# jopohl/urh

Hardware: NVIDIA H100
Metric: MSamples/s IQ demod+digitize (complex64) (higher is better)
Workload: dtype f32

## Files before the change

urh_b200/csrc/dense_f32.cuh:

```cuda
#pragma once
#include "dense.cuh"

struct SrcQad {
    static constexpr bool BINARY = false;
    template <typename T> __device__ __forceinline__ static int cls(T s, const UrhClassify& C, float) { return urh_classify((float)s, C); }
    template <typename T> __device__ __forceinline__ static void bits(T, const UrhClassify&, float, bool& nz, bool& ab) { nz = false; ab = false; }
    template <typename T> __device__ __forceinline__ static bool above(T, float) { return false; }
};
struct SrcQad2 {
    static constexpr bool BINARY = true;
    template <typename T> __device__ __forceinline__ static int cls(T s, const UrhClassify& C, float thr0) {
        const int c = ((float)s <= thr0) ? 0 : 1;
        return ((float)s == C.noise_value) ? -1 : c;
    }
    template <typename T> __device__ __forceinline__ static void bits(T s, const UrhClassify& C, float thr0, bool& nz, bool& ab) {
        nz = (float)s == C.noise_value;
        ab = !((float)s <= thr0) && !nz;
    }
    template <typename T> __device__ __forceinline__ static bool above(T s, float thr0) { return !((float)s <= thr0); }
};
struct SrcAbove {
    static constexpr bool BINARY = true;
    template <typename T> __device__ __forceinline__ static int cls(T s, const UrhClassify&, float thr0) { return (s > (T)thr0) ? 1 : 0; }
    template <typename T> __device__ __forceinline__ static void bits(T s, const UrhClassify&, float thr0, bool& nz, bool& ab) { nz = false; ab = s > (T)thr0; }
    template <typename T> __device__ __forceinline__ static bool above(T s, float thr0) { return s > (T)thr0; }
};
struct SrcCenter {
    static constexpr bool BINARY = true;
    template <typename T> __device__ __forceinline__ static int cls(T s, const UrhClassify&, float thr0) { return (s <= (T)thr0) ? 0 : 1; }
    template <typename T> __device__ __forceinline__ static void bits(T s, const UrhClassify&, float thr0, bool& nz, bool& ab) { nz = false; ab = !(s <= (T)thr0); }
    template <typename T> __device__ __forceinline__ static bool above(T s, float thr0) { return !(s <= (T)thr0); }
};

struct UrhSpec {
    const float* tg;
    float* margin;
    int64_t lo, hi;
    unsigned int* redone;
};

template <typename T> struct UrhVec2;
template <> struct UrhVec2<float> { typedef float2 type; };
template <> struct UrhVec2<double> { typedef double2 type; };

template <typename SRC, typename T>
__global__ void __launch_bounds__(URH_WARPS_PER_BLOCK * 32)
k_dense_f32(const T* __restrict__ x, int64_t n, int vec_in, const __grid_constant__ UrhClassify cls, int tol,
            UrhTileSummary* __restrict__ tiles, uint32_t* __restrict__ staging, int stage_cap,
            int16_t* __restrict__ init_cls, int cls_of_zero, const float* __restrict__ d_thr0 = nullptr,
            const UrhTileStats* __restrict__ tile_stats = nullptr, const UrhSpec spec = UrhSpec{}) {
    const float thr0 = d_thr0 ? *d_thr0 : cls.thr[0];
    if (d_thr0) cls_of_zero = (0.0f <= thr0) ? 0 : 1;
    const int lane = threadIdx.x & 31;
    const int64_t tile = (int64_t)blockIdx.x * URH_WARPS_PER_BLOCK + (threadIdx.x >> 5);
    const int64_t tile_start = tile * URH_TILE;
    if (tile_start >= n) return;
    const int tile_len = (int)((n - tile_start) < URH_TILE ? (n - tile_start) : URH_TILE);
    const int iters = (tile_len + 63) >> 6;
    if (tile_stats && tile_stats[tile].all_noise) {
        if (lane == 0) {
            UrhTileSummary s;
            s.first_cls = -1; s.last_cls = -1; s.head_len = tile_len; s.tail_len = tile_len; s.ncand = 0;
            tiles[tile] = s;
            if (tile_start == 0 && init_cls) *init_cls = (int16_t)-1;
        }
        return;
    }
    if (tile >= spec.lo && tile < spec.hi) {
        if (spec.margin[tile] > fabsf(__fsub_rn(thr0, *spec.tg))) return;
        if (lane == 0) atomicAdd(spec.redone, 1u);
    }
    UrhRunTracker rt;
    rt.init(tol, staging + tile * (int64_t)stage_cap);
    if (vec_in && tile_len == URH_TILE) {
        typedef typename UrhVec2<T>::type V;
        const V* p = (const V*)(x + tile_start) + lane;
        constexpr int ITERS = URH_TILE / 64;
        const bool no_noise = SRC::BINARY && tile_stats && cls.noise_value <= -4.0f && tile_stats[tile].cnt == URH_TILE;
        V cur[4], nxt[4];
#pragma unroll
        for (int j = 0; j < 4; j++) cur[j] = __ldg(p + j * 32);
        if (tile_start == 0 && lane == 0 && init_cls) *init_cls = (int16_t)(((float)cur[0].x == cls.noise_value) ? -1 : cls_of_zero);
        if (SRC::BINARY) {
            UrhTileResolve tr;
            tr.init();
#pragma unroll 1
            for (int it = 0; it < ITERS; it += 4) {
                if (it + 4 < ITERS) {
#pragma unroll
                    for (int j = 0; j < 4; j++) nxt[j] = __ldg(p + (it + 4 + j) * 32);
                }
                if (no_noise) {
#pragma unroll
                    for (int j = 0; j < 4; j++)
                        tr.keep(it + j, 0u, __ballot_sync(URH_FULL_MASK, SRC::template above<T>(cur[j].x, thr0)), 0u,
                                __ballot_sync(URH_FULL_MASK, SRC::template above<T>(cur[j].y, thr0)), lane);
                } else {
#pragma unroll
                    for (int j = 0; j < 4; j++) {
                        bool nx, ax, ny, ay;
                        SRC::template bits<T>(cur[j].x, cls, thr0, nx, ax);
                        SRC::template bits<T>(cur[j].y, cls, thr0, ny, ay);
                        tr.keep(it + j, __ballot_sync(URH_FULL_MASK, nx), __ballot_sync(URH_FULL_MASK, ax), __ballot_sync(URH_FULL_MASK, ny),
                                __ballot_sync(URH_FULL_MASK, ay), lane);
                    }
                }
#pragma unroll
                for (int j = 0; j < 4; j++) cur[j] = nxt[j];
            }
            tr.finish(tol, staging + tile * (int64_t)stage_cap, tiles + tile, lane);
            return;
        }
#pragma unroll 1
        for (int it = 0; it < ITERS; it += 4) {
            if (it + 4 < ITERS) {
#pragma unroll
                for (int j = 0; j < 4; j++) nxt[j] = __ldg(p + (it + 4 + j) * 32);
            }
#pragma unroll
            for (int j = 0; j < 4; j++)
                rt.feed(it + j, SRC::template cls<T>(cur[j].x, cls, thr0), SRC::template cls<T>(cur[j].y, cls, thr0), true, true, lane);
#pragma unroll
            for (int j = 0; j < 4; j++) cur[j] = nxt[j];
        }
        rt.finish(tile_len, tiles + tile, lane);
        return;
    }
    for (int it = 0; it < iters; it += 2) {
        T a0 = 0, a1 = 0, b0 = 0, b1 = 0;
        const int64_t pa = tile_start + (int64_t)it * 64 + 2 * lane;
        const int64_t pb = pa + 64;
        if (vec_in && pa + 1 < n) {
            const typename UrhVec2<T>::type v = __ldg((const typename UrhVec2<T>::type*)(x + pa));
            a0 = v.x; a1 = v.y;
        } else {
            if (pa < n) a0 = __ldg(x + pa);
            if (pa + 1 < n) a1 = __ldg(x + pa + 1);
        }
        const bool has_b = it + 1 < iters;
        if (has_b) {
            if (vec_in && pb + 1 < n) {
                const typename UrhVec2<T>::type v = __ldg((const typename UrhVec2<T>::type*)(x + pb));
                b0 = v.x; b1 = v.y;
            } else {
                if (pb < n) b0 = __ldg(x + pb);
                if (pb + 1 < n) b1 = __ldg(x + pb + 1);
            }
        }
        if (pa == 0 && init_cls) *init_cls = (int16_t)(((float)a0 == cls.noise_value) ? -1 : cls_of_zero);
        rt.feed(it, SRC::template cls<T>(a0, cls, thr0), SRC::template cls<T>(a1, cls, thr0), pa < n, pa + 1 < n, lane);
        if (has_b) rt.feed(it + 1, SRC::template cls<T>(b0, cls, thr0), SRC::template cls<T>(b1, cls, thr0), pb < n, pb + 1 < n, lane);
    }
    rt.finish(tile_len, tiles + tile, lane);
}
```

urh_b200/csrc/digitize.cu:

```cuda
#include "dense.cuh"
#include "scan.cuh"
#include "sparse.cuh"
#ifndef URH_FAST_MIN_BLOCKS
#define URH_FAST_MIN_BLOCKS 4
#endif
#include "fsk_fast.cuh"
#include "dense_f32.cuh"
#include "stream_ring.cuh"

#include <math.h>
#include <stdlib.h>


template <int DT, int MOD, bool DIGITIZE>
__device__ __forceinline__ void dense_iq_tile(const void* __restrict__ iq, int64_t n, const UrhDemodParams& dp, float* __restrict__ qad_out,
                                              int vec_in, int vec_out, const UrhClassify& cls, int tol, UrhTileSummary* __restrict__ tiles,
                                              uint32_t* __restrict__ staging, int stage_cap, int16_t* __restrict__ init_cls, int cls_of_zero,
                                              int64_t tile, int has_halo, UrhTileStats* __restrict__ tile_stats, const UrhFine& fine,
                                              unsigned int* s_fine, unsigned int* g_fine) {
    const int lane = threadIdx.x & 31;
    const int64_t tile_start = tile * URH_TILE;
    const int tile_len = (int)((n - tile_start) < URH_TILE ? (n - tile_start) : URH_TILE);
    const int iters = (tile_len + 63) >> 6;

// ... 874 lines not shown
        const StreamSizes z = stream_sizes(n, dtype, tolerance, sc->chunk_samples, sc->ring, URH_STREAM_ENTRY_DEMOD_CENTER_DIGITIZE);
        scs = z.cs;
        URH_CHECK(ring.init(ctx, sc->ring, sc->ring * r256(z.src_slot)));
        const int64_t slot = r256(z.src_slot);
        URH_CHECK(stream_run(ctx, n, scs, ring, (const char*)sc->h_iq, urh_iq_bytes(dtype), true, ring.mem, slot, sc->h_qad, d_qad_out,
                             [&](int64_t, int64_t s0, int64_t s1, int s) {
                                 return stream_dense_iq<false>(ctx, dtype, mod_type, ring.mem, slot, n, dp, d_qad_out, cls, 0, nullptr, s0, s1, s,
                                                               ts, fine);
                             }, true));
    }
    cls.noise_value = urh_noise_value(mod_type);
    cls.order = 2;
    const int tol = tolerance;
    const int cap = stage_cap_for(tol);
    UrhTileSummary* tiles = nullptr;
    uint32_t* staging = nullptr;
    int16_t* d_init = nullptr;
    if (!sc) {
        URH_CHECK(urh_arena(ctx, (size_t)ntiles, &tiles));
        URH_CHECK(urh_arena(ctx, (size_t)ntiles * cap, &staging));
        URH_CHECK(urh_arena(ctx, 8, &d_init));
    }
    const bool speculate = !sharded && !h_iq && !sc && mod_type == URH_MOD_FSK && dtype == URH_DT_F32 &&
                           getenv("URH_B200_NO_SPECULATE") == nullptr;
    UrhSpec spec = {};
    if (speculate) {
        float* tg;
        URH_CHECK(urh_arena(ctx, 1, &tg));
        URH_CHECK(urh_arena(ctx, 1, &spec.redone));
        URH_CHECK(urh_arena(ctx, (size_t)ntiles, &spec.margin));
        spec.tg = tg;
        const char* forced = getenv("URH_B200_SPECULATE_GUESS");
        URH_LAUNCH(ctx, k_speculate_guess, 1, URH_GUESS_THREADS, 0, (const float2*)d_iq, n, dp.noise_sqrd, forced ? 1 : 0,
                   forced ? strtof(forced, nullptr) : 0.0f, tg, spec.redone);
    }
    int chunk_no = 0;
    for (int64_t t0 = 0; t0 < (sc ? 0 : ntiles); t0 += chunk_tiles, chunk_no++) {
        const int64_t t1 = (t0 + chunk_tiles < ntiles) ? t0 + chunk_tiles : ntiles;
        if (h_iq) {
            const int64_t s0 = t0 * URH_TILE, s1 = (t1 * URH_TILE < n) ? t1 * URH_TILE : n;
            cudaEvent_t ev = ctx->ev_copy[chunk_no & 1];
            URH_CUDA(ctx, cudaMemcpyAsync((char*)d_iq + (size_t)s0 * sample_bytes, (const char*)h_iq + (size_t)s0 * sample_bytes,
                                          (size_t)(s1 - s0) * sample_bytes, cudaMemcpyHostToDevice, ctx->copy_stream[0]));
            URH_CUDA(ctx, cudaEventRecord(ev, ctx->copy_stream[0]));
            URH_CUDA(ctx, cudaStreamWaitEvent(ctx->stream, ev, 0));
        }
        if (mod_type == URH_MOD_ASK)
            URH_CHECK((launch_dense_iq_m<URH_MOD_ASK, false>(ctx, dtype, d_iq, n, dp, d_qad_out, cls, 0, nullptr, nullptr, 0, nullptr, 0, has_halo, ts, t0, t1, fine)));
        else
            URH_CHECK((launch_dense_iq_m<URH_MOD_FSK, false>(ctx, dtype, d_iq, n, dp, d_qad_out, cls, tol, tiles, staging, cap, nullptr, 0, has_halo,
                                                             ts, t0, t1, fine, speculate ? &spec : nullptr)));
    }
    CenterPlan* plan = nullptr;
    URH_CHECK(urh_center_chain(ctx, d_qad_out, n, ts, max_size, sharded ? ctx->nccl_rank : 0, sharded ? ctx->nccl_world : 1,
                               fine.gh ? &fine : nullptr, &plan));
    const float* d_centerf;
    const double* d_center;
    const int* d_state;
    urh_center_plan_result(ctx, plan, &d_centerf, &d_center, &d_state);
    int64_t rows = 0;
    if (sc) {
        URH_CUDA(ctx, cudaMemcpyAsync(ctx->h_mail + 40, d_center, sizeof(double), cudaMemcpyDeviceToHost, ctx->stream));
        URH_CUDA(ctx, cudaMemcpyAsync(ctx->h_mail + 41, d_state, sizeof(int), cudaMemcpyDeviceToHost, ctx->stream));
        URH_CHECK(urh_center_plan_certify_stats(ctx, plan, ctx->h_mail + 42));
        URH_CUDA(ctx, cudaMemcpyAsync(ctx->h_mail + 45, (const int64_t*)ctx->center_prefix + ntiles, sizeof(int64_t), cudaMemcpyDeviceToHost,
                                      ctx->stream));
        URH_CUDA(ctx, cudaStreamSynchronize(ctx->stream));
        int st0 = 0;
        memcpy(&st0, ctx->h_mail + 41, sizeof(int));
        if (st0 == 1) {
            StreamDigitizer dz;
            URH_CHECK(dz.init(ctx, n, scs, tol, mod_type == URH_MOD_ASK, samples_per_symbol));
            for (int64_t s0 = 0; s0 < n; s0 += scs) {
                const int64_t s1 = s0 + scs < n ? s0 + scs : n;
                URH_CHECK(stream_dense_qad(ctx, d_qad_out + s0, s0, s1, cls, dz, d_centerf, ts));
                URH_CHECK(dz.finish(ctx, s0, s1));
            }
            rows = dz.rows;
        }
        *sc->kept = ctx->h_mail[45];
    } else {
        URH_CUDA(ctx, cudaMemsetAsync(d_init, 0, 16, ctx->stream));
        const int vec_in = (((uintptr_t)d_qad_out % 8) == 0) ? 1 : 0;
        URH_LAUNCH(ctx, (k_dense_f32<SrcQad2, float>), (unsigned)urh_div_up(ntiles, URH_WARPS_PER_BLOCK), URH_WARPS_PER_BLOCK * 32, 0,
                   (const float*)d_qad_out, n, vec_in, cls, tol, tiles, staging, cap, d_init, 0, d_centerf, (const UrhTileStats*)ts, spec);
        URH_CUDA(ctx, cudaMemcpyAsync(ctx->h_mail + 40, d_center, sizeof(double), cudaMemcpyDeviceToHost, ctx->stream));
        URH_CUDA(ctx, cudaMemcpyAsync(ctx->h_mail + 41, d_state, sizeof(int), cudaMemcpyDeviceToHost, ctx->stream));
        URH_CHECK(urh_center_plan_certify_stats(ctx, plan, ctx->h_mail + 42));
        ctx->h_mail[46] = 0;
        if (speculate) URH_CUDA(ctx, cudaMemcpyAsync(ctx->h_mail + 46, spec.redone, sizeof(unsigned int), cudaMemcpyDeviceToHost, ctx->stream));
        if (sharded)
            URH_CHECK(urh_finish_shard(ctx, n, tol, mod_type == URH_MOD_ASK, samples_per_symbol, tiles, staging, cap, d_init, global_offset, n_total, &rows));
        else
            URH_CHECK(urh_finish_local(ctx, n, tol, mod_type == URH_MOD_ASK, samples_per_symbol, tiles, staging, cap, d_init, &rows));
    }
    memcpy(center, ctx->h_mail + 40, sizeof(double));
    int st = 0;
    memcpy(&st, ctx->h_mail + 41, sizeof(int));
    *center_state = st;
    ctx->center_cert[0] = ctx->h_mail[42];
    ctx->center_cert[1] = fine.gh ? URH_FINE_NB : 0;
    ctx->center_cert[2] = ctx->h_mail[44];
    const int64_t redone = (spec.hi > spec.lo) ? ctx->h_mail[46] : 0;
    ctx->spec_stats[0] = spec.hi - spec.lo;
    ctx->spec_stats[1] = spec.hi - spec.lo - redone;
    ctx->spec_stats[2] = redone;
    if (st != 1) {
        ctx->pulses_k = 0;
        rows = 0;
    }
    *k = rows;
    return URH_OK;
}

extern "C" int urh_speculate_stats(urh_ctx* ctx, int64_t* h_out3) {
    for (int i = 0; i < 3; i++) h_out3[i] = ctx->spec_stats[i];
    return URH_OK;
}

extern "C" int urh_demod_center_digitize(urh_ctx* ctx, const void* d_iq, int dtype, int64_t n, float noise_mag, int mod_type,
                                         uint16_t tolerance, uint32_t samples_per_symbol, int64_t max_size, float* d_qad_out,
                                         double* center, int* center_state, int64_t* k) {
    return demod_center_digitize_impl(ctx, d_iq, dtype, n, 0, noise_mag, mod_type, tolerance, samples_per_symbol, max_size, d_qad_out, false,
                                      0, n, center, center_state, k);
}

extern "C" int urh_demod_center_digitize_host(urh_ctx* ctx, const void* h_iq, int dtype, int64_t n, float noise_mag, int mod_type,
                                              uint16_t tolerance, uint32_t samples_per_symbol, int64_t max_size, int64_t chunk_samples,
                                              void* d_iq_scratch, float* d_qad_out, double* center, int* center_state, int64_t* k) {
    if (!h_iq || !d_iq_scratch) return URH_ERR_INVALID;
    URH_CUDA(ctx, cudaEventRecord(ctx->ev_comp[0], ctx->stream));
    URH_CUDA(ctx, cudaStreamWaitEvent(ctx->copy_stream[0], ctx->ev_comp[0], 0));
    return demod_center_digitize_impl(ctx, d_iq_scratch, dtype, n, 0, noise_mag, mod_type, tolerance, samples_per_symbol, max_size, d_qad_out,
                                      false, 0, n, center, center_state, k, h_iq, chunk_samples > 0 ? chunk_samples : ((int64_t)1 << 24));
}

extern "C" int urh_shard_demod_center_digitize_host(urh_ctx* ctx, const void* h_iq, int dtype, int64_t n, int has_halo, float noise_mag,
                                                    int mod_type, uint16_t tolerance, uint32_t samples_per_symbol, int64_t max_size,
                                                    int64_t chunk_samples, void* d_iq_scratch, float* d_qad_out, int64_t global_offset,
                                                    int64_t n_total, double* center, int* center_state, int64_t* k) {
    if (!h_iq || !d_iq_scratch) return URH_ERR_INVALID;
    URH_CUDA(ctx, cudaEventRecord(ctx->ev_comp[0], ctx->stream));
    URH_CUDA(ctx, cudaStreamWaitEvent(ctx->copy_stream[0], ctx->ev_comp[0], 0));
    return demod_center_digitize_impl(ctx, d_iq_scratch, dtype, n, has_halo, noise_mag, mod_type, tolerance, samples_per_symbol, max_size,
                                      d_qad_out, true, global_offset, n_total, center, center_state, k, h_iq,
                                      chunk_samples > 0 ? chunk_samples : ((int64_t)1 << 24));
}

extern "C" int urh_shard_demod_center_digitize(urh_ctx* ctx, const void* d_iq, int dtype, int64_t n, int has_halo, float noise_mag,
                                               int mod_type, uint16_t tolerance, uint32_t samples_per_symbol, int64_t max_size,
                                               float* d_qad_out, int64_t global_offset, int64_t n_total, double* center,
                                               int* center_state, int64_t* k) {
    return demod_center_digitize_impl(ctx, d_iq, dtype, n, has_halo, noise_mag, mod_type, tolerance, samples_per_symbol, max_size, d_qad_out,
                                      true, global_offset, n_total, center, center_state, k);
}

extern "C" int urh_afp_demod_stream(urh_ctx* ctx, const void* h_iq, int dtype, int64_t n, float noise_mag, int mod_type, int64_t chunk_samples,
                                    int ring, float* h_qad) {
    if (!h_iq || !h_qad) return URH_ERR_INVALID;
    URH_CHECK(stream_check(ctx, n, ring, mod_type, dtype, true));
    urh_arena_reset(ctx);
    const StreamSizes z = stream_sizes(n, dtype, 0, chunk_samples, ring, URH_STREAM_ENTRY_AFP_DEMOD);
    StreamRing R;
    URH_CHECK(R.init(ctx, ring, z.ring_bytes));
    char* d_src = R.mem;
    float* d_qad = (float*)(R.mem + ring * r256(z.src_slot));
    const UrhDemodParams dp = make_demod_params(noise_mag, mod_type, dtype);
// ... 276 lines not shown
```

urh_b200/csrc/finish.cu:

```cuda
#include "sparse.cuh"
#include "tilescan.cuh"

#include <limits.h>

#define CLS_NONE INT_MIN

struct __align__(16) CandAgg {
    int64_t cnt;
    int32_t last_cls;
    int32_t pad;
};
struct CandOp {
    __device__ __forceinline__ CandAgg operator()(const CandAgg& a, const CandAgg& b) const {
        CandAgg r;
        r.cnt = a.cnt + b.cnt;
        r.last_cls = (b.last_cls != CLS_NONE) ? b.last_cls : a.last_cls;
        r.pad = 0;
        return r;
    }
};
struct __align__(16) FireAgg {
    int64_t fired;
    int64_t last_pos;
};
struct FireOp {
    __device__ __forceinline__ FireAgg operator()(const FireAgg& a, const FireAgg& b) const {
        FireAgg r;
        r.fired = a.fired + b.fired;
        r.last_pos = (b.last_pos >= 0) ? b.last_pos : a.last_pos;
        return r;
    }
};

struct ScanRunCarry {
    const UrhTileSummary* tiles;
    int64_t n;
    RunCarry* carry;
    __device__ __forceinline__ RunCarry load(int64_t t) const {
        const int64_t rem = n - t * URH_TILE;
        const int tile_len = rem < URH_TILE ? (int)rem : URH_TILE;
        const UrhTileSummary s = tiles[t];
        RunCarry r;
        r.len = s.tail_len;
        r.cls = s.last_cls;
        r.flags = (s.head_len == tile_len) ? 1 : 0;
        return r;
    }
    __device__ __forceinline__ void post(int64_t t, const RunCarry& excl, const RunCarry&) const { carry[t] = excl; }
};

struct ScanCandidates {
    const UrhTileSummary* tiles;
    const uint32_t* staging;
    int stage_cap;
    const RunCarry* carry;
    const RunCarry* xcarry;
    int tol;
    int32_t* head_rel;
    int32_t* prev_cls;
    __device__ __forceinline__ CandAgg load(int64_t t) const {
        const UrhTileSummary s = tiles[t];
        RunCarry c = carry[t];
        if (xcarry) c = RunCarryOp()(*xcarry, c);
        int64_t start_len = 0;
        if (!(c.flags & 2) && c.cls == s.first_cls) start_len = c.len;
        int32_t rel = -1;
        if (start_len <= tol && (int64_t)tol < start_len + s.head_len) rel = (int32_t)(tol - start_len);
        head_rel[t] = rel;
        CandAgg r;
        r.cnt = (int64_t)s.ncand + (rel >= 0 ? 1 : 0);
        r.last_cls = CLS_NONE;
        if (s.ncand > 0) r.last_cls = (int32_t)(staging[t * (int64_t)stage_cap + s.ncand - 1] & 0xffffu) - 1;
        else if (rel >= 0) r.last_cls = s.first_cls;
        r.pad = 0;
        return r;
    }
    __device__ __forceinline__ void post(int64_t t, const CandAgg& excl, const CandAgg&) const { prev_cls[t] = excl.last_cls; }
};

struct ScanFirings {
    const UrhTileSummary* tiles;
    const uint32_t* staging;
    int stage_cap;
    const int32_t* head_rel;
    const int32_t* prev_cls;
    const int16_t* d_prev0;
    int64_t global_offset;
    int64_t* row_off;
    int64_t* prev_fired;
    __device__ __forceinline__ FireAgg load(int64_t t) const {
        const UrhTileSummary s = tiles[t];
        int prev = prev_cls[t];
        if (prev == CLS_NONE) prev = *d_prev0;
        const int64_t base = t * URH_TILE + global_offset;
        FireAgg r;
        r.fired = 0;
        r.last_pos = -1;
        const int32_t rel = head_rel[t];
        if (rel >= 0) {
            const int c = s.first_cls;
            if (c != prev) { r.fired++; r.last_pos = base + rel; }
            prev = c;
        }
        const uint32_t* st = staging + t * (int64_t)stage_cap;
        for (int j = 0; j < s.ncand; j++) {
            const uint32_t v = st[j];
            const int c = (int)(v & 0xffffu) - 1;
            if (c != prev) { r.fired++; r.last_pos = base + (v >> 16); }
            prev = c;
        }
        return r;
    }
    __device__ __forceinline__ void post(int64_t t, const FireAgg& excl, const FireAgg&) const {
        row_off[t] = excl.fired;
        prev_fired[t] = excl.last_pos;
    }
};

__global__ void __launch_bounds__(256) k_finish_rows(const UrhTileSummary* __restrict__ tiles, const uint32_t* __restrict__ staging,
                                                    int stage_cap, const int32_t* __restrict__ head_rel, const int32_t* __restrict__ prev_cls,
                                                    const int16_t* __restrict__ d_prev0, const int64_t* __restrict__ row_off,
                                                    const int64_t* __restrict__ prev_fired, const int64_t* __restrict__ d_xprev_fired,
                                                    int64_t ntiles, int64_t global_offset, int64_t n_total, int tol, int is_ask, int64_t sps,
                                                    int emit_tail, int64_t row_base, int64_t* __restrict__ out, int64_t cap_rows,
                                                    int64_t* __restrict__ d_out) {
    const int64_t t = (int64_t)blockIdx.x * blockDim.x + threadIdx.x;
    if (t >= ntiles) return;
    const UrhTileSummary s = tiles[t];
    int prev = prev_cls[t];
    if (prev == CLS_NONE) prev = *d_prev0;
    int64_t pp = prev_fired[t];
    if (pp < 0) pp = *d_xprev_fired;
    int64_t idx = row_off[t];
    const int64_t base = t * URH_TILE + global_offset;
    auto fire = [&](int64_t p, int c) {
        if (c != prev) {
            const int64_t rec = (pp >= 0) ? (p - pp) : (p + 1 - tol);
            int64_t st = prev;
            if (is_ask && st == -1 && rec < sps) st = 0;
            if (idx < cap_rows) *((longlong2*)out + idx) = make_longlong2(st, rec);
            idx++;
            pp = p;
        }
        prev = c;
    };
    const int32_t rel = head_rel[t];
    if (rel >= 0) fire(base + rel, s.first_cls);
    const uint32_t* st = staging + t * (int64_t)stage_cap;
    for (int j = 0; j < s.ncand; j++) {
        const uint32_t v = st[j];
        fire(base + (v >> 16), (int)(v & 0xffffu) - 1);
    }
    if (t == ntiles - 1) {
        const int64_t fired = idx;
        if (emit_tail && (is_ask || row_base + fired < n_total)) {
            if (idx < cap_rows) *((longlong2*)out + idx) = make_longlong2(prev, (pp >= 0) ? (n_total - 1 - pp) : (n_total - tol));
            idx++;
        }
        d_out[0] = idx;
        d_out[1] = fired;
    }
}

struct ScanMergeRows {
    const int64_t* raw;
    int64_t rows;
    int64_t n_total;
    int has_tail;
    int64_t* out;
    int64_t* d_k;
    const int64_t* prev_last;
    int64_t row_base;
    __device__ __forceinline__ int64_t load(int64_t r) const {
        if (r == 0) return (prev_last && raw[0] == *prev_last) ? 0 : 1;
        return raw[2 * r] != raw[2 * r - 2] ? 1 : 0;
    }
    __device__ __forceinline__ void post(int64_t r, const int64_t& excl, const int64_t& head) const {
        const bool is_tail = has_tail && r == rows - 1;
        if (is_tail && row_base + excl >= n_total) {
            *d_k = excl;
            return;
        }
        const int64_t o = excl + head - 1;
        if (head) out[2 * o] = raw[2 * r];
        atomicAdd((unsigned long long*)&out[2 * o + 1], (unsigned long long)raw[2 * r + 1]);
        if (r == rows - 1) *d_k = o + 1;
    }
};
struct AddI64 {
    __device__ __forceinline__ int64_t operator()(int64_t a, int64_t b) const { return a + b; }
};

__global__ void k_pack_stage1(const int16_t* __restrict__ d_init, const RunCarry* __restrict__ total, int64_t* __restrict__ msg) {
    memcpy(msg, total, sizeof(RunCarry));
    msg[2] = *d_init;
    msg[3] = 0;
}
__global__ void k_fold_carry(const int64_t* __restrict__ all, int rank, RunCarry* __restrict__ xcarry) {
    RunCarry acc;
    acc.len = 0; acc.cls = 0; acc.flags = 2 | 1;
    for (int q = 0; q < rank; q++) {
        RunCarry c;
        memcpy(&c, all + 4 * q, sizeof(c));
        acc = RunCarryOp()(acc, c);
    }
    if (rank == 0) acc.flags = 2;
    else acc.flags &= ~1;
    *xcarry = acc;
}
__global__ void k_fold_prev_cls(const int64_t* __restrict__ all, int rank, const int64_t* __restrict__ stage1, int16_t* __restrict__ prev0) {
    int v = (int)stage1[2];
    for (int q = 0; q < rank; q++) {
        CandAgg c;
        memcpy(&c, all + 2 * q, sizeof(c));
        if (c.last_cls != CLS_NONE) v = c.last_cls;
    }
    *prev0 = (int16_t)v;
}
__global__ void k_fold_prev_fired(const int64_t* __restrict__ all, int rank, int64_t* __restrict__ xprev) {
    int64_t v = -1;
    for (int q = 0; q < rank; q++) {
        FireAgg c;
        memcpy(&c, all + 2 * q, sizeof(c));
        if (c.last_pos >= 0) v = c.last_pos;
    }
    *xprev = v;
}

__global__ void k_chain_start(const int16_t* __restrict__ d_init, UrhChain* __restrict__ chain) {
    chain->run.len = 0; chain->run.cls = 0; chain->run.flags = 2 | 1;
    chain->prev_fired = -1;
    chain->last_state = INT64_MIN;
    chain->prev_cls = *d_init;
}
__global__ void k_chain_advance(UrhChain* __restrict__ chain, const RunCarry* __restrict__ tot_run, const CandAgg* __restrict__ tot_cand,
                                const FireAgg* __restrict__ tot_fire) {
    chain->run = RunCarryOp()(chain->run, *tot_run);
    if (tot_cand->last_cls != CLS_NONE) chain->prev_cls = (int16_t)tot_cand->last_cls;
    if (tot_fire->last_pos >= 0) chain->prev_fired = tot_fire->last_pos;
}
__global__ void k_chain_last_row(UrhChain* __restrict__ chain, const int64_t* __restrict__ table, int64_t rows) {
    if (rows > 0) chain->last_state = table[2 * (rows - 1)];
}

int urh_coll_allgather(urh_ctx* ctx, const void* d_send, void* d_recv, size_t bytes_per_rank);
extern "C" int urh_p2p_check(urh_ctx* ctx);

struct FinishShard {
    int rank, world;
    int64_t global_offset;
    int64_t n_total;
    int emit_tail;
    UrhChain* chain;
    int64_t row_base, rows_cap;
};

static int finish_tiles(urh_ctx* ctx, int64_t n, int tol, bool is_ask, uint32_t sps, const UrhTileSummary* tiles, const uint32_t* staging,
                        int stage_cap, const int16_t* d_init, const FinishShard& sh, int64_t* k) {
    const int64_t ntiles = urh_div_up(n, URH_TILE);
    const bool sharded = sh.world > 1;
    UrhChain* chain = sh.chain;
    RunCarry* carry;
    int32_t *head_rel, *prev_cls;
    int64_t *row_off, *prev_fired, *d_small;
    URH_CHECK(urh_arena(ctx, (size_t)ntiles, &carry));
    URH_CHECK(urh_arena(ctx, (size_t)ntiles, &head_rel));
    URH_CHECK(urh_arena(ctx, (size_t)ntiles, &prev_cls));
    URH_CHECK(urh_arena(ctx, (size_t)ntiles, &row_off));
    URH_CHECK(urh_arena(ctx, (size_t)ntiles, &prev_fired));
    URH_CHECK(urh_arena(ctx, (size_t)(32 + 8 * (sharded ? sh.world : 0)), &d_small));
    URH_CUDA(ctx, cudaMemsetAsync(d_small, 0xff, 4 * sizeof(int64_t), ctx->stream));
    RunCarry* d_tot_run = (RunCarry*)(d_small + 4);
    CandAgg* d_tot_cand = (CandAgg*)(d_small + 6);
    FireAgg* d_tot_fire = (FireAgg*)(d_small + 8);
    RunCarry* d_xcarry = (RunCarry*)(d_small + 10);
    int16_t* d_prev0 = (int16_t*)(d_small + 12);
    int64_t* d_xprev = d_small + 13;
    int64_t* d_msg1 = d_small + 16;
    int64_t* d_all1 = d_small + 32;
    int64_t* d_all2 = d_all1 + 4 * (sharded ? sh.world : 0);
    int64_t* d_all3 = d_all2 + 2 * (sharded ? sh.world : 0);

    if (chain && sh.global_offset == 0) URH_LAUNCH(ctx, k_chain_start, 1, 1, 0, d_init, chain);
    RunCarry rc_ident;
    rc_ident.len = 0; rc_ident.cls = 0; rc_ident.flags = 2 | 1;
    ScanRunCarry fa;
    fa.tiles = tiles; fa.n = n; fa.carry = carry;
    URH_CHECK((urhts::scan<RunCarry, RunCarryOp, ScanRunCarry>(ctx, ntiles, rc_ident, RunCarryOp(), fa, d_tot_run)));
    if (sharded) {
        URH_LAUNCH(ctx, k_pack_stage1, 1, 1, 0, d_init, (const RunCarry*)d_tot_run, d_msg1);
        URH_TL_MARK(ctx, "x4 run carry: enter");
        URH_CHECK(urh_coll_allgather(ctx, d_msg1, d_all1, 4 * sizeof(int64_t)));
        URH_TL_MARK(ctx, "x4 run carry: done");
        URH_LAUNCH(ctx, k_fold_carry, 1, 1, 0, (const int64_t*)d_all1, sh.rank, d_xcarry);
    }
    ScanCandidates fb;
    fb.tiles = tiles; fb.staging = staging; fb.stage_cap = stage_cap; fb.carry = carry;
    fb.xcarry = sharded ? d_xcarry : (chain ? &chain->run : nullptr);
    fb.tol = tol; fb.head_rel = head_rel; fb.prev_cls = prev_cls;
    CandAgg ca_ident;
    ca_ident.cnt = 0; ca_ident.last_cls = CLS_NONE; ca_ident.pad = 0;
    URH_CHECK((urhts::scan<CandAgg, CandOp, ScanCandidates>(ctx, ntiles, ca_ident, CandOp(), fb, d_tot_cand)));
    const int16_t* prev0 = chain ? &chain->prev_cls : d_init;
    if (sharded) {
        URH_TL_MARK(ctx, "x5 candidates: enter");
        URH_CHECK(urh_coll_allgather(ctx, d_tot_cand, d_all2, sizeof(CandAgg)));
        URH_TL_MARK(ctx, "x5 candidates: done");
        URH_LAUNCH(ctx, k_fold_prev_cls, 1, 1, 0, (const int64_t*)d_all2, sh.rank, (const int64_t*)d_all1, d_prev0);
        prev0 = d_prev0;
    }
    ScanFirings fc;
    fc.tiles = tiles; fc.staging = staging; fc.stage_cap = stage_cap; fc.head_rel = head_rel; fc.prev_cls = prev_cls; fc.d_prev0 = prev0;
    fc.global_offset = sh.global_offset; fc.row_off = row_off; fc.prev_fired = prev_fired;
    FireAgg fi_ident;
    fi_ident.fired = 0; fi_ident.last_pos = -1;
    URH_CHECK((urhts::scan<FireAgg, FireOp, ScanFirings, 4>(ctx, ntiles, fi_ident, FireOp(), fc, d_tot_fire)));
    const int64_t* xprev = chain ? &chain->prev_fired : d_small + 2;
    if (sharded) {
        URH_TL_MARK(ctx, "x6 firings: enter");
        URH_CHECK(urh_coll_allgather(ctx, d_tot_fire, d_all3, sizeof(FireAgg)));
        URH_TL_MARK(ctx, "x6 firings: done");
        URH_LAUNCH(ctx, k_fold_prev_fired, 1, 1, 0, (const int64_t*)d_all3, sh.rank, d_xprev);
        xprev = d_xprev;
    }

    int64_t cap_rows = (int64_t)ctx->pulses_cap_rows;
    const int64_t guess = n / 64 + 1024;
    if (!chain && cap_rows < guess) {
        URH_CHECK(urh_ensure_pulses(ctx, (size_t)guess));
        cap_rows = (int64_t)ctx->pulses_cap_rows;
    }
    const int64_t row_base = chain ? sh.row_base : 0;
    int64_t* raw = ctx->pulses + 2 * row_base;
    int64_t raw_cap = chain ? sh.rows_cap : cap_rows;
    if (is_ask) URH_CHECK(urh_arena(ctx, (size_t)raw_cap * 2, &raw));
    int64_t got[2] = {0, 0};
    for (int attempt = 0; attempt < 2; attempt++) {
        URH_LAUNCH(ctx, k_finish_rows, (unsigned)urh_div_up(ntiles, 256), 256, 0, tiles, staging, stage_cap, (const int32_t*)head_rel,
                   (const int32_t*)prev_cls, prev0, (const int64_t*)row_off, (const int64_t*)prev_fired, xprev, ntiles, sh.global_offset,
                   sh.n_total, tol, is_ask ? 1 : 0, (int64_t)sps, sh.emit_tail, row_base, raw, raw_cap, d_small);
        if (sharded && attempt == 0) URH_TL_MARK(ctx, "rows written");
        URH_CHECK(urh_read_i64(ctx, d_small, 2, got));
        if (sharded) URH_CHECK(urh_p2p_check(ctx));
        if (got[0] <= raw_cap) break;
        if (attempt == 1 || chain) URH_FAIL(ctx, URH_ERR_CUDA, "finish_tiles: row buffer overflow after regrowth");
        if (is_ask) {
            URH_CHECK(urh_arena(ctx, (size_t)got[0] * 2, &raw));
            raw_cap = got[0];
        } else {
            URH_CHECK(urh_ensure_pulses(ctx, (size_t)got[0]));
            raw = ctx->pulses;
            raw_cap = (int64_t)ctx->pulses_cap_rows;
        }
    }
    if (chain) URH_LAUNCH(ctx, k_chain_advance, 1, 1, 0, chain, (const RunCarry*)d_tot_run, (const CandAgg*)d_tot_cand, (const FireAgg*)d_tot_fire);
    int64_t K = got[0];
    if (is_ask && K > 0) {
        if (!chain) URH_CHECK(urh_ensure_pulses(ctx, (size_t)K));
        int64_t* out = ctx->pulses + 2 * row_base;
        URH_CUDA(ctx, cudaMemsetAsync(out, 0, (size_t)K * 2 * sizeof(int64_t), ctx->stream));
        ScanMergeRows fm;
        fm.raw = raw; fm.rows = K; fm.n_total = sh.n_total; fm.has_tail = (sh.emit_tail && K > got[1]) ? 1 : 0; fm.out = out;
        fm.d_k = d_small;
        fm.prev_last = (chain && row_base > 0) ? &chain->last_state : nullptr;
        fm.row_base = row_base;
        URH_CHECK((urhts::scan<int64_t, AddI64, ScanMergeRows>(ctx, K, (int64_t)0, AddI64(), fm, (int64_t*)nullptr)));
        URH_CHECK(urh_read_i64(ctx, d_small, 1, &K));
        if (chain) URH_LAUNCH(ctx, k_chain_last_row, 1, 1, 0, chain, (const int64_t*)ctx->pulses, row_base + K);
    }
    ctx->pulses_k = row_base + K;
    *k = K;
    return URH_OK;
}

int urh_finish_chunk(urh_ctx* ctx, int64_t n, int tol, bool is_ask, uint32_t sps, const UrhTileSummary* tiles, const uint32_t* staging,
                     int stage_cap, const int16_t* d_init, UrhChain* chain, int64_t global_offset, int64_t n_total, int64_t row_base,
                     int64_t rows_cap, int64_t* k) {
    FinishShard sh;
    sh.rank = 0; sh.world = 1; sh.global_offset = global_offset; sh.n_total = n_total;
    sh.emit_tail = (global_offset + n == n_total) ? 1 : 0;
    sh.chain = chain; sh.row_base = row_base; sh.rows_cap = rows_cap;
    return finish_tiles(ctx, n, tol, is_ask, sps, tiles, staging, stage_cap, d_init, sh, k);
}

int urh_finish_local(urh_ctx* ctx, int64_t n, int tol, bool is_ask, uint32_t sps, const UrhTileSummary* tiles, const uint32_t* staging,
                     int stage_cap, const int16_t* d_init, int64_t* k) {
    FinishShard sh;
    sh.rank = 0; sh.world = 1; sh.global_offset = 0; sh.n_total = n; sh.emit_tail = 1;
    sh.chain = nullptr; sh.row_base = 0; sh.rows_cap = 0;
    return finish_tiles(ctx, n, tol, is_ask, sps, tiles, staging, stage_cap, d_init, sh, k);
}

int urh_finish_shard(urh_ctx* ctx, int64_t n, int tol, bool is_ask, uint32_t sps, const UrhTileSummary* tiles, const uint32_t* staging,
                     int stage_cap, const int16_t* d_init, int64_t global_offset, int64_t n_total, int64_t* k) {
    FinishShard sh;
    sh.rank = ctx->nccl_rank; sh.world = ctx->nccl_world; sh.global_offset = global_offset; sh.n_total = n_total;
    sh.emit_tail = (ctx->nccl_rank == ctx->nccl_world - 1) ? 1 : 0;
    sh.chain = nullptr; sh.row_base = 0; sh.rows_cap = 0;
    return finish_tiles(ctx, n, tol, is_ask, sps, tiles, staging, stage_cap, d_init, sh, k);
}
```

Before: 204,100.

## Restructure dense classify and finish passes for warp-cooperative tile processing

The dense f32 classifier becomes a grid-stride, warp-ballot loop. It skips all-noise and speculated tiles per lane before running the tile body, and when speculating it caps the grid at resident occupancy. The candidates scan now precomputes a per-tile firing summary, so the firings scan only reads that compact record and no longer walks the staging buffer again. The row-finishing kernel maps one warp to 32 tiles and walks candidates cooperatively with shuffles and ballots instead of one thread per tile. This trades extra scratch memory and more complex code for less serial per-thread work and fewer repeated reads of staging.

Result: faster. 214,300 (median of 6 runs) (+5.0%).

```diff
diff --git a/urh_b200/csrc/dense_f32.cuh b/urh_b200/csrc/dense_f32.cuh
--- a/urh_b200/csrc/dense_f32.cuh
+++ b/urh_b200/csrc/dense_f32.cuh
@@ -44,32 +44,13 @@
 template <> struct UrhVec2<double> { typedef double2 type; };
 
 template <typename SRC, typename T>
-__global__ void __launch_bounds__(URH_WARPS_PER_BLOCK * 32)
-k_dense_f32(const T* __restrict__ x, int64_t n, int vec_in, const __grid_constant__ UrhClassify cls, int tol,
-            UrhTileSummary* __restrict__ tiles, uint32_t* __restrict__ staging, int stage_cap,
-            int16_t* __restrict__ init_cls, int cls_of_zero, const float* __restrict__ d_thr0 = nullptr,
-            const UrhTileStats* __restrict__ tile_stats = nullptr, const UrhSpec spec = UrhSpec{}) {
-    const float thr0 = d_thr0 ? *d_thr0 : cls.thr[0];
-    if (d_thr0) cls_of_zero = (0.0f <= thr0) ? 0 : 1;
-    const int lane = threadIdx.x & 31;
-    const int64_t tile = (int64_t)blockIdx.x * URH_WARPS_PER_BLOCK + (threadIdx.x >> 5);
+__device__ __forceinline__ void dense_f32_tile(const T* __restrict__ x, int64_t n, int vec_in, const UrhClassify& cls, float thr0, int tol,
+                                               UrhTileSummary* __restrict__ tiles, uint32_t* __restrict__ staging, int stage_cap,
+                                               int16_t* __restrict__ init_cls, int cls_of_zero, const UrhTileStats* __restrict__ tile_stats,
+                                               int64_t tile, int lane) {
     const int64_t tile_start = tile * URH_TILE;
-    if (tile_start >= n) return;
     const int tile_len = (int)((n - tile_start) < URH_TILE ? (n - tile_start) : URH_TILE);
     const int iters = (tile_len + 63) >> 6;
-    if (tile_stats && tile_stats[tile].all_noise) {
-        if (lane == 0) {
-            UrhTileSummary s;
-            s.first_cls = -1; s.last_cls = -1; s.head_len = tile_len; s.tail_len = tile_len; s.ncand = 0;
-            tiles[tile] = s;
-            if (tile_start == 0 && init_cls) *init_cls = (int16_t)-1;
-        }
-        return;
-    }
-    if (tile >= spec.lo && tile < spec.hi) {
-        if (spec.margin[tile] > fabsf(__fsub_rn(thr0, *spec.tg))) return;
-        if (lane == 0) atomicAdd(spec.redone, 1u);
-    }
     UrhRunTracker rt;
     rt.init(tol, staging + tile * (int64_t)stage_cap);
     if (vec_in && tile_len == URH_TILE) {
@@ -153,3 +134,35 @@
     }
     rt.finish(tile_len, tiles + tile, lane);
 }
+
+template <typename SRC, typename T>
+__global__ void __launch_bounds__(URH_WARPS_PER_BLOCK * 32)
+k_dense_f32(const T* __restrict__ x, int64_t n, int vec_in, const __grid_constant__ UrhClassify cls, int tol,
+            UrhTileSummary* __restrict__ tiles, uint32_t* __restrict__ staging, int stage_cap,
+            int16_t* __restrict__ init_cls, int cls_of_zero, const float* __restrict__ d_thr0 = nullptr,
+            const UrhTileStats* __restrict__ tile_stats = nullptr, const UrhSpec spec = UrhSpec{}) {
+    const float thr0 = d_thr0 ? *d_thr0 : cls.thr[0];
+    if (d_thr0) cls_of_zero = (0.0f <= thr0) ? 0 : 1;
+    const int lane = threadIdx.x & 31;
+    const int64_t ntiles = urh_div_up(n, URH_TILE);
+    const int64_t stride = (int64_t)gridDim.x * URH_WARPS_PER_BLOCK;
+    for (int64_t t0 = (int64_t)blockIdx.x * URH_WARPS_PER_BLOCK + (threadIdx.x >> 5); t0 < ntiles; t0 += 32 * stride) {
+        const int64_t mine = t0 + lane * stride;
+        bool work = mine < ntiles;
+        if (work && tile_stats && tile_stats[mine].all_noise) {
+            const int64_t rem = n - mine * URH_TILE;
+            const int tile_len = rem < URH_TILE ? (int)rem : URH_TILE;
+            UrhTileSummary s;
+            s.first_cls = -1; s.last_cls = -1; s.head_len = tile_len; s.tail_len = tile_len; s.ncand = 0;
+            tiles[mine] = s;
+            if (mine == 0 && init_cls) *init_cls = (int16_t)-1;
+            work = false;
+        } else if (work && mine >= spec.lo && mine < spec.hi) {
+            if (spec.margin[mine] > fabsf(__fsub_rn(thr0, *spec.tg))) work = false;
+            else atomicAdd(spec.redone, 1u);
+        }
+        for (unsigned m = __ballot_sync(URH_FULL_MASK, work); m; m &= m - 1)
+            dense_f32_tile<SRC, T>(x, n, vec_in, cls, thr0, tol, tiles, staging, stage_cap, init_cls, cls_of_zero, tile_stats,
+                                   t0 + (int64_t)(__ffs(m) - 1) * stride, lane);
+    }
+}
diff --git a/urh_b200/csrc/digitize.cu b/urh_b200/csrc/digitize.cu
--- a/urh_b200/csrc/digitize.cu
+++ b/urh_b200/csrc/digitize.cu
@@ -980,7 +980,14 @@
     } else {
         URH_CUDA(ctx, cudaMemsetAsync(d_init, 0, 16, ctx->stream));
         const int vec_in = (((uintptr_t)d_qad_out % 8) == 0) ? 1 : 0;
-        URH_LAUNCH(ctx, (k_dense_f32<SrcQad2, float>), (unsigned)urh_div_up(ntiles, URH_WARPS_PER_BLOCK), URH_WARPS_PER_BLOCK * 32, 0,
+        int64_t grid = urh_div_up(ntiles, URH_WARPS_PER_BLOCK);
+        if (speculate) {
+            int per_sm = 0;
+            URH_CUDA(ctx, cudaOccupancyMaxActiveBlocksPerMultiprocessor(&per_sm, k_dense_f32<SrcQad2, float>, URH_WARPS_PER_BLOCK * 32, 0));
+            const int64_t resident = (int64_t)ctx->sm_count * (per_sm > 0 ? per_sm : 1);
+            if (grid > resident) grid = resident;
+        }
+        URH_LAUNCH(ctx, (k_dense_f32<SrcQad2, float>), (unsigned)grid, URH_WARPS_PER_BLOCK * 32, 0,
                    (const float*)d_qad_out, n, vec_in, cls, tol, tiles, staging, cap, d_init, 0, d_centerf, (const UrhTileStats*)ts, spec);
         URH_CUDA(ctx, cudaMemcpyAsync(ctx->h_mail + 40, d_center, sizeof(double), cudaMemcpyDeviceToHost, ctx->stream));
         URH_CUDA(ctx, cudaMemcpyAsync(ctx->h_mail + 41, d_state, sizeof(int), cudaMemcpyDeviceToHost, ctx->stream));
diff --git a/urh_b200/csrc/finish.cu b/urh_b200/csrc/finish.cu
--- a/urh_b200/csrc/finish.cu
+++ b/urh_b200/csrc/finish.cu
@@ -49,6 +49,12 @@
     __device__ __forceinline__ void post(int64_t t, const RunCarry& excl, const RunCarry&) const { carry[t] = excl; }
 };
 
+struct __align__(16) TileFire {
+    int32_t first_cls;
+    int32_t first_rel;
+    int32_t fired;
+    int32_t last_rel;
+};
 struct ScanCandidates {
     const UrhTileSummary* tiles;
     const uint32_t* staging;
@@ -58,6 +64,7 @@
     int tol;
     int32_t* head_rel;
     int32_t* prev_cls;
+    TileFire* fire;
     __device__ __forceinline__ CandAgg load(int64_t t) const {
         const UrhTileSummary s = tiles[t];
         RunCarry c = carry[t];
@@ -67,11 +74,39 @@
         int32_t rel = -1;
         if (start_len <= tol && (int64_t)tol < start_len + s.head_len) rel = (int32_t)(tol - start_len);
         head_rel[t] = rel;
+        TileFire f;
+        f.first_cls = CLS_NONE; f.first_rel = -1; f.fired = 0; f.last_rel = -1;
+        int prev = CLS_NONE;
+        if (rel >= 0) {
+            prev = s.first_cls;
+            f.first_cls = prev;
+            f.first_rel = rel;
+        }
+        const uint32_t* st = staging + t * (int64_t)stage_cap;
+        for (int j = 0; j < s.ncand; j += 4) {
+            uint32_t w[4];
+#pragma unroll
+            for (int u = 0; u < 4; u++) w[u] = (j + u < s.ncand) ? st[j + u] : 0u;
+#pragma unroll
+            for (int u = 0; u < 4; u++) {
+                if (j + u < s.ncand) {
+                    const int cl = (int)(w[u] & 0xffffu) - 1;
+                    const int p = (int)(w[u] >> 16);
+                    if (prev == CLS_NONE) {
+                        f.first_cls = cl;
+                        f.first_rel = p;
+                    } else if (cl != prev) {
+                        f.fired++;
+                        f.last_rel = p;
+                    }
+                    prev = cl;
+                }
+            }
+        }
+        fire[t] = f;
         CandAgg r;
         r.cnt = (int64_t)s.ncand + (rel >= 0 ? 1 : 0);
-        r.last_cls = CLS_NONE;
-        if (s.ncand > 0) r.last_cls = (int32_t)(staging[t * (int64_t)stage_cap + s.ncand - 1] & 0xffffu) - 1;
-        else if (rel >= 0) r.last_cls = s.first_cls;
+        r.last_cls = prev;
         r.pad = 0;
         return r;
     }
@@ -79,36 +114,24 @@
 };
 
 struct ScanFirings {
-    const UrhTileSummary* tiles;
-    const uint32_t* staging;
-    int stage_cap;
-    const int32_t* head_rel;
+    const TileFire* fire;
     const int32_t* prev_cls;
     const int16_t* d_prev0;
     int64_t global_offset;
     int64_t* row_off;
     int64_t* prev_fired;
     __device__ __forceinline__ FireAgg load(int64_t t) const {
-        const UrhTileSummary s = tiles[t];
+        const TileFire f = fire[t];
         int prev = prev_cls[t];
         if (prev == CLS_NONE) prev = *d_prev0;
-        const int64_t base = t * URH_TILE + global_offset;
         FireAgg r;
-        r.fired = 0;
-        r.last_pos = -1;
-        const int32_t rel = head_rel[t];
-        if (rel >= 0) {
-            const int c = s.first_cls;
-            if (c != prev) { r.fired++; r.last_pos = base + rel; }
-            prev = c;
-        }
-        const uint32_t* st = staging + t * (int64_t)stage_cap;
-        for (int j = 0; j < s.ncand; j++) {
-            const uint32_t v = st[j];
-            const int c = (int)(v & 0xffffu) - 1;
-            if (c != prev) { r.fired++; r.last_pos = base + (v >> 16); }
-            prev = c;
-        }
+        r.fired = f.fired;
+        int32_t last = f.last_rel;
+        if (f.first_cls != CLS_NONE && f.first_cls != prev) {
+            r.fired++;
+            if (last < 0) last = f.first_rel;
+        }
+        r.last_pos = (last >= 0) ? t * URH_TILE + global_offset + last : -1;
         return r;
     }
     __device__ __forceinline__ void post(int64_t t, const FireAgg& excl, const FireAgg&) const {
@@ -116,6 +139,45 @@
         prev_fired[t] = excl.last_pos;
     }
 };
+
+constexpr int FIN_TILES = 32;
+constexpr int FIN_BATCH = 8;
+
+struct FinRows {
+    int64_t* out;
+    int64_t cap_rows;
+    int tol;
+    int is_ask;
+    int64_t sps;
+};
+
+struct FinWalk {
+    int prev;
+    int64_t pp;
+    int64_t idx;
+};
+
+__device__ __forceinline__ void fin_row(const FinRows& R, int64_t idx, int64_t p, int64_t pp, int prev) {
+    const int64_t rec = (pp >= 0) ? (p - pp) : (p + 1 - R.tol);
+    int64_t st = prev;
+    if (R.is_ask && st == -1 && rec < R.sps) st = 0;
+    if (idx < R.cap_rows) *((longlong2*)R.out + idx) = make_longlong2(st, rec);
+}
+
+__device__ __forceinline__ void fin_chunk(FinWalk& W, uint32_t w, int cnt, int lane, int64_t base, const FinRows& R) {
+    const int c = (int)(w & 0xffffu) - 1;
+    const int rel = (int)(w >> 16);
+    int pc = __shfl_up_sync(URH_FULL_MASK, c, 1);
+    if (lane == 0) pc = W.prev;
+    const bool fire = lane < cnt && c != pc;
+    const unsigned fm = __ballot_sync(URH_FULL_MASK, fire);
+    const unsigned lower = fm & ((1u << lane) - 1u);
+    const int before = __shfl_sync(URH_FULL_MASK, rel, lower ? 31 - __clz(lower) : 0);
+    if (fire) fin_row(R, W.idx + __popc(lower), base + rel, lower ? base + before : W.pp, pc);
+    if (fm) W.pp = base + __shfl_sync(URH_FULL_MASK, rel, 31 - __clz(fm));
+    W.idx += __popc(fm);
+    if (cnt > 0) W.prev = __shfl_sync(URH_FULL_MASK, c, cnt - 1);
+}
 
 __global__ void __launch_bounds__(256) k_finish_rows(const UrhTileSummary* __restrict__ tiles, const uint32_t* __restrict__ staging,
                                                     int stage_cap, const int32_t* __restrict__ head_rel, const int32_t* __restrict__ prev_cls,
@@ -124,41 +186,69 @@
                                                     int64_t ntiles, int64_t global_offset, int64_t n_total, int tol, int is_ask, int64_t sps,
                                                     int emit_tail, int64_t row_base, int64_t* __restrict__ out, int64_t cap_rows,
                                                     int64_t* __restrict__ d_out) {
-    const int64_t t = (int64_t)blockIdx.x * blockDim.x + threadIdx.x;
-    if (t >= ntiles) return;
-    const UrhTileSummary s = tiles[t];
-    int prev = prev_cls[t];
-    if (prev == CLS_NONE) prev = *d_prev0;
-    int64_t pp = prev_fired[t];
-    if (pp < 0) pp = *d_xprev_fired;
-    int64_t idx = row_off[t];
-    const int64_t base = t * URH_TILE + global_offset;
-    auto fire = [&](int64_t p, int c) {
-        if (c != prev) {
-            const int64_t rec = (pp >= 0) ? (p - pp) : (p + 1 - tol);
-            int64_t st = prev;
-            if (is_ask && st == -1 && rec < sps) st = 0;
-            if (idx < cap_rows) *((longlong2*)out + idx) = make_longlong2(st, rec);
-            idx++;
-            pp = p;
-        }
-        prev = c;
-    };
-    const int32_t rel = head_rel[t];
-    if (rel >= 0) fire(base + rel, s.first_cls);
-    const uint32_t* st = staging + t * (int64_t)stage_cap;
-    for (int j = 0; j < s.ncand; j++) {
-        const uint32_t v = st[j];
-        fire(base + (v >> 16), (int)(v & 0xffffu) - 1);
-    }
-    if (t == ntiles - 1) {
-        const int64_t fired = idx;
-        if (emit_tail && (is_ask || row_base + fired < n_total)) {
-            if (idx < cap_rows) *((longlong2*)out + idx) = make_longlong2(prev, (pp >= 0) ? (n_total - 1 - pp) : (n_total - tol));
-            idx++;
-        }
-        d_out[0] = idx;
-        d_out[1] = fired;
+    const int64_t t0 = ((int64_t)blockIdx.x * blockDim.x + threadIdx.x) / 32 * FIN_TILES;
+    if (t0 >= ntiles) return;
+    const int lane = threadIdx.x & 31;
+    FinRows R;
+    R.out = out; R.cap_rows = cap_rows; R.tol = tol; R.is_ask = is_ask; R.sps = sps;
+    const int64_t tl = t0 + lane;
+    int l_first = 0, l_ncand = 0, l_rel = -1, l_prev = 0;
+    int64_t l_idx = 0, l_pp = -1;
+    if (tl < ntiles) {
+        const UrhTileSummary s = tiles[tl];
+        l_first = s.first_cls;
+        l_ncand = s.ncand;
+        l_rel = head_rel[tl];
+        l_prev = prev_cls[tl];
+        if (l_prev == CLS_NONE) l_prev = *d_prev0;
+        l_idx = row_off[tl];
+        l_pp = prev_fired[tl];
+        if (l_pp < 0) l_pp = *d_xprev_fired;
+    }
+    for (int j0 = 0; j0 < FIN_TILES && t0 + j0 < ntiles; j0 += FIN_BATCH) {
+        uint32_t w0[FIN_BATCH];
+#pragma unroll
+        for (int u = 0; u < FIN_BATCH; u++) {
+            const int nc = __shfl_sync(URH_FULL_MASK, l_ncand, j0 + u);
+            w0[u] = (lane < nc) ? __ldg(staging + (t0 + j0 + u) * (int64_t)stage_cap + lane) : 0u;
+        }
+#pragma unroll
+        for (int u = 0; u < FIN_BATCH; u++) {
+            const int j = j0 + u;
+            const int64_t t = t0 + j;
+            if (t >= ntiles) break;
+            const int64_t base = t * URH_TILE + global_offset;
+            const int ncand = __shfl_sync(URH_FULL_MASK, l_ncand, j);
+            const int rel = __shfl_sync(URH_FULL_MASK, l_rel, j);
+            FinWalk W;
+            W.prev = __shfl_sync(URH_FULL_MASK, l_prev, j);
+            W.pp = __shfl_sync(URH_FULL_MASK, l_pp, j);
+            W.idx = __shfl_sync(URH_FULL_MASK, l_idx, j);
+            if (rel >= 0) {
+                const int c = __shfl_sync(URH_FULL_MASK, l_first, j);
+                if (c != W.prev) {
+                    if (lane == 0) fin_row(R, W.idx, base + rel, W.pp, W.prev);
+                    W.idx++;
+                    W.pp = base + rel;
+                }
+                W.prev = c;
+            }
+            const uint32_t* st = staging + t * (int64_t)stage_cap;
+            for (int k = 0; k < ncand; k += 32) {
+                const uint32_t w = (k == 0) ? w0[u] : ((k + lane < ncand) ? __ldg(st + k + lane) : 0u);
+                fin_chunk(W, w, min(32, ncand - k), lane, base, R);
+            }
+            if (t == ntiles - 1 && lane == 0) {
+                int64_t idx = W.idx;
+                const int64_t fired = idx;
+                if (emit_tail && (is_ask || row_base + fired < n_total)) {
+                    if (idx < cap_rows) *((longlong2*)out + idx) = make_longlong2(W.prev, (W.pp >= 0) ? (n_total - 1 - W.pp) : (n_total - tol));
+                    idx++;
+                }
+                d_out[0] = idx;
+                d_out[1] = fired;
+            }
+        }
     }
 }
 
@@ -268,6 +358,8 @@
     URH_CHECK(urh_arena(ctx, (size_t)ntiles, &prev_cls));
     URH_CHECK(urh_arena(ctx, (size_t)ntiles, &row_off));
     URH_CHECK(urh_arena(ctx, (size_t)ntiles, &prev_fired));
+    TileFire* fire;
+    URH_CHECK(urh_arena(ctx, (size_t)ntiles, &fire));
     URH_CHECK(urh_arena(ctx, (size_t)(32 + 8 * (sharded ? sh.world : 0)), &d_small));
     URH_CUDA(ctx, cudaMemsetAsync(d_small, 0xff, 4 * sizeof(int64_t), ctx->stream));
     RunCarry* d_tot_run = (RunCarry*)(d_small + 4);
@@ -297,10 +389,10 @@
     ScanCandidates fb;
     fb.tiles = tiles; fb.staging = staging; fb.stage_cap = stage_cap; fb.carry = carry;
     fb.xcarry = sharded ? d_xcarry : (chain ? &chain->run : nullptr);
-    fb.tol = tol; fb.head_rel = head_rel; fb.prev_cls = prev_cls;
+    fb.tol = tol; fb.head_rel = head_rel; fb.prev_cls = prev_cls; fb.fire = fire;
     CandAgg ca_ident;
     ca_ident.cnt = 0; ca_ident.last_cls = CLS_NONE; ca_ident.pad = 0;
-    URH_CHECK((urhts::scan<CandAgg, CandOp, ScanCandidates>(ctx, ntiles, ca_ident, CandOp(), fb, d_tot_cand)));
+    URH_CHECK((urhts::scan<CandAgg, CandOp, ScanCandidates, 4>(ctx, ntiles, ca_ident, CandOp(), fb, d_tot_cand)));
     const int16_t* prev0 = chain ? &chain->prev_cls : d_init;
     if (sharded) {
         URH_TL_MARK(ctx, "x5 candidates: enter");
@@ -310,11 +402,11 @@
         prev0 = d_prev0;
     }
     ScanFirings fc;
-    fc.tiles = tiles; fc.staging = staging; fc.stage_cap = stage_cap; fc.head_rel = head_rel; fc.prev_cls = prev_cls; fc.d_prev0 = prev0;
-    fc.global_offset = sh.global_offset; fc.row_off = row_off; fc.prev_fired = prev_fired;
+    fc.fire = fire; fc.prev_cls = prev_cls; fc.d_prev0 = prev0; fc.global_offset = sh.global_offset; fc.row_off = row_off;
+    fc.prev_fired = prev_fired;
     FireAgg fi_ident;
     fi_ident.fired = 0; fi_ident.last_pos = -1;
-    URH_CHECK((urhts::scan<FireAgg, FireOp, ScanFirings, 4>(ctx, ntiles, fi_ident, FireOp(), fc, d_tot_fire)));
+    URH_CHECK((urhts::scan<FireAgg, FireOp, ScanFirings>(ctx, ntiles, fi_ident, FireOp(), fc, d_tot_fire)));
     const int64_t* xprev = chain ? &chain->prev_fired : d_small + 2;
     if (sharded) {
         URH_TL_MARK(ctx, "x6 firings: enter");
@@ -336,7 +428,7 @@
     if (is_ask) URH_CHECK(urh_arena(ctx, (size_t)raw_cap * 2, &raw));
     int64_t got[2] = {0, 0};
     for (int attempt = 0; attempt < 2; attempt++) {
-        URH_LAUNCH(ctx, k_finish_rows, (unsigned)urh_div_up(ntiles, 256), 256, 0, tiles, staging, stage_cap, (const int32_t*)head_rel,
+        URH_LAUNCH(ctx, k_finish_rows, (unsigned)urh_div_up(ntiles, 8 * FIN_TILES), 256, 0, tiles, staging, stage_cap, (const int32_t*)head_rel,
                    (const int32_t*)prev_cls, prev0, (const int64_t*)row_off, (const int64_t*)prev_fired, xprev, ntiles, sh.global_offset,
                    sh.n_total, tol, is_ask ? 1 : 0, (int64_t)sps, sh.emit_tail, row_base, raw, raw_cap, d_small);
         if (sharded && attempt == 0) URH_TL_MARK(ctx, "rows written");
```
